# tinh2044/SCAttenNet

Measured on AMD Instinct MI355X. Metric: clips/sec fwd+bwd, (B=8,T=256,K=79,d=256) at 1/2/4/8 MI355X, higher is better.
Workload: dtype fp32; 1 GPU; cfg2: 4-stream SCA (mapping + 4x self / causal / cross-merge), B=8 T=256 K=79 d=256 H=16, fwd+bwd all params; clips_per_gpu=8, frames=256, joints=79, d_model=256, heads=16, layers=4, hipgraph=True, parallelism=dp1, devices=1

## Files before the change

### scattennet_amd/csrc/gemm.hip

```cpp
#include <stdlib.h>

#include <type_traits>
#include "common.h"
#include "../../include/scatten.h"

namespace {

constexpr int KPAD = 4;

struct GemmArgs {
  sca_gemm_problem p[SCA_GEMM_MAX_PROBLEMS];
  int splitk;
  float* ws;
  const unsigned long long* drop_off;
  long slab_off[SCA_GEMM_MAX_PROBLEMS];
  long bias_off[SCA_GEMM_MAX_PROBLEMS];
  unsigned* counters;
  int nprob;
  int flat;
  int tile_beg[SCA_GEMM_MAX_PROBLEMS + 1];
};

template <int BM_, int BN_, int WM_, int WN_, int BK_, int STAGES_>
struct Cfg {
// ... 1094 lines not shown
#pragma unroll
    for (int r = 0; r < 4; ++r)
#pragma unroll
      for (int i = 0; i < 4; ++i) {
        const int m = m0 + wm + 16 * g + 4 * r + i;
        if (m < P.M && ncol) {
          const f32x4 x = f32x4{acc[i][0][r], acc[i][1][r], acc[i][2][r], acc[i][3][r]} * alpha;
          const int off = (int)(((long)ks * MN + (long)m * P.N + n) * 4);
          if (fused_k) __builtin_amdgcn_raw_buffer_store_b128(*reinterpret_cast<const u32x4*>(&x), rs, off, 0, 16);
          else __builtin_amdgcn_raw_buffer_store_b128(*reinterpret_cast<const u32x4*>(&x), rs, off, 0, 0);
        }
      }
    if (!fused_k) return;
    asm volatile("s_waitcnt vmcnt(0)" ::: "memory");
    __syncthreads();
    unsigned* cnt = args.counters + (long)pid * gx * gy + (long)by * gx + bx;
    if (tid == 0)
      flag = __hip_atomic_fetch_add(cnt, 1u, __ATOMIC_RELAXED, __HIP_MEMORY_SCOPE_AGENT) == (unsigned)(splitk - 1);
    __syncthreads();
    if (!flag) return;
    if (tid == 0) __hip_atomic_store(cnt, 0u, __ATOMIC_RELAXED, __HIP_MEMORY_SCOPE_AGENT);
    __builtin_amdgcn_fence(__ATOMIC_ACQUIRE, "wavefront");
    if (P.bias_grad && bx == 0 && tid < TB_BM && m0 + tid < P.M) {
      float* bp = args.ws + args.bias_off[pid] + m0 + tid;
      float t = 0.f;
      for (int s2 = 0; s2 < splitk; ++s2)
        t += __hip_atomic_load(bp + (long)s2 * P.M, __ATOMIC_RELAXED, __HIP_MEMORY_SCOPE_AGENT);
      P.bias_grad[m0 + tid] = t * P.bias_grad_scale;
    }
    if (!ncol) return;
    DropMask dm;
    if (P.epi & SCA_EPI_DROPOUT) dm.init(P.drop_seed, P.drop_p, args.drop_off);
#pragma unroll 4
    for (int q = 0; q < 16; ++q) {
      const int m = m0 + wm + 16 * g + q;
      if (m >= P.M) continue;
      const long e = (long)m * P.N + n;
      f32x4 t = ld4_sc1(rs, e);
      for (int s2 = 1; s2 < splitk; ++s2) t += ld4_sc1(rs, s2 * MN + e);
      epilogue_piece(P, t, m, n, dm);
    }
    return;
  }
  if (!ncol) return;
  DropMask dm;
  if (P.epi & SCA_EPI_DROPOUT) dm.init(P.drop_seed, P.drop_p, args.drop_off);
#pragma unroll
  for (int r = 0; r < 4; ++r)
#pragma unroll
    for (int i = 0; i < 4; ++i) {
      const int m = m0 + wm + 16 * g + 4 * r + i;
      if (m < P.M)
        epilogue_piece(P, f32x4{acc[i][0][r], acc[i][1][r], acc[i][2][r], acc[i][3][r]} * alpha, m, n, dm);
    }
}

constexpr int NB_LD = TB_BK + 4;
constexpr int NB_OP = TB_BM * NB_LD;

template <bool INTER, int NPRE, bool B_KN, bool ILV = false, int TM = 128>
__global__ __launch_bounds__(256, 1) void gemm_ntb_kernel(const GemmArgs args) {
  constexpr int WT = TM / 2, NQ = WT / 16, NJ = TM / 16;
  constexpr int OP = TM * NB_LD;
  __shared__ __attribute__((aligned(16))) float lds[2 * OP];
  if constexpr (B_KN && SCA_CRIT_PRIO > 0) __builtin_amdgcn_s_setprio(SCA_CRIT_PRIO);

  const unsigned gx = gridDim.x, gy = gridDim.y;
  const unsigned nwg = gx * gy * gridDim.z;
  const unsigned orig = blockIdx.x + gx * (blockIdx.y + gy * blockIdx.z);
  const unsigned xcd = orig & 7, q8 = nwg >> 3, r8 = nwg & 7;
  const unsigned wgid = (xcd < r8 ? xcd * (q8 + 1) : r8 * (q8 + 1) + (xcd - r8) * q8) + (orig >> 3);
  const int bx = wgid % gx, by = (wgid / gx) % gy, pid = wgid / (gx * gy);
  const sca_gemm_problem& P = args.p[pid];
  const int m0 = by * TM, n0 = bx * TM;
  if (m0 >= P.M || n0 >= P.N) return;

  const int tid = threadIdx.x, lane = tid & 63, wave = tid >> 6;
  const int kg = lane >> 4, li = lane & 15;
  const int wm = (wave >> 1) * WT, wn = (wave & 1) * WT;
  const int nseg = P.nseg;
  const int it0 = P.seg[0].K / TB_BK, it1 = nseg > 1 ? P.seg[1].K / TB_BK : 0;
  const int nit = it0 + it1 + (nseg > 2 ? P.seg[2].K / TB_BK : 0);

  const int srow = tid >> 4, sk4 = 4 * (tid & 15);
  f32x4 st[2 * NJ];
  auto load = [&](int it) {
    int s = 0, lit = it;
    if (lit >= it0) {
      lit -= it0;
      s = 1;
      if (lit >= it1) {
        lit -= it1;
        s = 2;
      }
    }
    const sca_gemm_seg& G = P.seg[s];
    const __amdgpu_buffer_rsrc_t ra = __builtin_amdgcn_make_buffer_rsrc(
        const_cast<float*>(G.A), 0, (int)(((long)(P.M - 1) * G.lda + G.K) * 4), 0x00020000);
    const __amdgpu_buffer_rsrc_t rb = __builtin_amdgcn_make_buffer_rsrc(
        const_cast<float*>(G.B), 0,
        (int)((B_KN ? (long)(G.K - 1) * G.ldb + P.N : (long)(P.N - 1) * G.ldb + G.K) * 4), 0x00020000);
#pragma unroll
    for (int j = 0; j < NJ; ++j) {
      st[j] = tb_load(ra, (int)(((long)min(m0 + srow + 16 * j, P.M - 1) * G.lda + sk4) * 4), lit * TB_BK * 4);
      if constexpr (B_KN) {
        const int b = NJ * wave + j;
        const int k = 16 * (b & 3) + li, c4 = 4 * (4 * (b >> 2) + kg);
        st[NJ + j] = tb_load(rb, (int)(((long)k * G.ldb + min(n0 + c4, P.N - 4)) * 4), lit * TB_BK * G.ldb * 4);
      } else {
        st[NJ + j] = tb_load(rb, (int)(((long)min(n0 + srow + 16 * j, P.N - 1) * G.ldb + sk4) * 4), lit * TB_BK * 4);
      }
    }
  };
  float* wbase = lds + srow * NB_LD + sk4;
  auto store = [&]() {
#pragma unroll
    for (int j = 0; j < NJ; ++j) {
      st4(wbase + j * 16 * NB_LD, st[j]);
      if constexpr (B_KN) {
        const int b = NJ * wave + j;
        const int k = 16 * (b & 3) + li, c4 = 4 * (4 * (b >> 2) + kg);
#pragma unroll
        for (int q = 0; q < 4; ++q) lds[OP + (c4 + q) * NB_LD + k] = st[NJ + j][q];
      } else {
        st4(wbase + OP + j * 16 * NB_LD, st[NJ + j]);
      }
    }
  };

  f32x4 acc[NQ][NQ];
#pragma unroll
  for (int i = 0; i < NQ; ++i)
#pragma unroll
    for (int j = 0; j < NQ; ++j) acc[i][j] = f32x4{0.f, 0.f, 0.f, 0.f};

  const float* ra_lds = lds + (wm + li) * NB_LD + 4 * kg;
  const float* rb_lds = lds + OP + (wn + li) * NB_LD + 4 * kg;
  auto iter = [&](auto wr_c, auto ld_c, int it) {
    constexpr bool WR = decltype(wr_c)::value, LD = decltype(ld_c)::value;
    f32x4 a[4][NQ], b[4][NQ];
#pragma unroll
    for (int kc = 0; kc < 4; ++kc)
#pragma unroll
      for (int q = 0; q < NQ; ++q) {
        a[kc][q] = ld4(ra_lds + 16 * q * NB_LD + 16 * kc);
        b[kc][q] = ld4(rb_lds + 16 * q * NB_LD + 16 * kc);
      }
    auto steps = [&](int t0, int t1) {
#pragma unroll
      for (int t = t0; t < t1; ++t)
#pragma unroll
        for (int i = 0; i < NQ; ++i)
#pragma unroll
          for (int j = 0; j < NQ; ++j) acc[i][j] = mfma16(a[t >> 2][i][t & 3], b[t >> 2][j][t & 3], acc[i][j]);
    };
    steps(0, NPRE);
    if constexpr (ILV) ilv_read<0, 8, NQ, NPRE * NQ * NQ / 8>();
    if constexpr (INTER) __builtin_amdgcn_sched_barrier(0);
    __syncthreads();
    if constexpr (INTER) __builtin_amdgcn_sched_barrier(0);
    if constexpr (WR) {
      store();
      if constexpr (LD) load(it + 2);
    }
    steps(NPRE, 16);
    if constexpr (ILV && WR) ilv_store<0, 2 * NJ, B_KN ? 3 : 1, (16 - NPRE) * NQ * NQ / (2 * NJ)>();
    __syncthreads();
  };
  load(0);
  store();
  if (nit > 1) load(1);
  __syncthreads();
  int it = 0;
#pragma unroll 1
  for (; it + 2 < nit; ++it) iter(std::true_type{}, std::true_type{}, it);
  if (it + 1 < nit) iter(std::true_type{}, std::false_type{}, it++);
  if (it < nit) iter(std::false_type{}, std::false_type{}, it);

  constexpr int LR = WT / 4;
  float* img = lds + wave * WT * NB_LD;
  const float alpha = P.seg[0].alpha;
#pragma unroll
  for (int i = 0; i < NQ; ++i)
#pragma unroll
    for (int j = 0; j < NQ; ++j)
#pragma unroll
      for (int r = 0; r < 4; ++r) img[(16 * i + 4 * kg + r) * NB_LD + 16 * j + li] = acc[i][j][r] * alpha;
  __builtin_amdgcn_fence(__ATOMIC_RELEASE, "wavefront");
  __builtin_amdgcn_wave_barrier();
  __builtin_amdgcn_fence(__ATOMIC_ACQUIRE, "wavefront");
  const int n = n0 + wn + 4 * (lane % LR);
  if (n >= P.N) return;
  DropMask dm;
  if (P.epi & SCA_EPI_DROPOUT) dm.init(P.drop_seed, P.drop_p, args.drop_off);
#pragma unroll 4
  for (int q = 0; q < WT * LR / 64; ++q) {
    const int rho = lane / LR + (64 / LR) * q, m = m0 + wm + rho;
    if (m < P.M) epilogue_piece(P, ld4(img + rho * NB_LD + 4 * (lane % LR)), m, n, dm);
  }
}

constexpr int LR_SMEM = (32 + 256) * 68 * 4;
template <bool B_KN>
__device__ __forceinline__ void ln_rows_reg(const sca_gemm_problem& P, int m0, float* lds, f32x4 (&acc)[2][2]) {
  constexpr int LD = 68, NPRE = 4;
  const int tid = threadIdx.x, lane = tid & 63, wave = tid >> 6, kg = lane >> 4, li = lane & 15;
  float* Ai = lds;
  float* Bi = lds + 32 * LD;
  const int nseg = P.nseg;
  const int it0 = P.seg[0].K / 64, it1 = nseg > 1 ? P.seg[1].K / 64 : 0;
  const int nit = it0 + it1 + (nseg > 2 ? P.seg[2].K / 64 : 0);
  const int arow = tid >> 4, ak4 = 4 * (tid & 15);
  f32x4 st[9];
  auto load = [&](int it) {
    int sg = 0, lit = it;
    if (lit >= it0) {
      lit -= it0;
      sg = 1;
      if (lit >= it1) {
        lit -= it1;
        sg = 2;
      }
    }
    const sca_gemm_seg& G = P.seg[sg];
    const __amdgpu_buffer_rsrc_t ra = __builtin_amdgcn_make_buffer_rsrc(
        const_cast<float*>(G.A), 0, (int)(((long)(P.M - 1) * G.lda + G.K) * 4), 0x00020000);
    const __amdgpu_buffer_rsrc_t rb = __builtin_amdgcn_make_buffer_rsrc(
        const_cast<float*>(G.B), 0,
        (int)((B_KN ? (long)(G.K - 1) * G.ldb + P.N : (long)(P.N - 1) * G.ldb + G.K) * 4), 0x00020000);
    st[0] = tb_load(ra, (int)(((long)min(m0 + arow, P.M - 1) * G.lda + ak4) * 4), lit * 256);
#pragma unroll
    for (int j = 0; j < 8; ++j) {
      if constexpr (B_KN) {
        const int b = 8 * wave + j, k = 16 * (b & 3) + li, c4 = 4 * (4 * (b >> 2) + kg);
        st[1 + j] = tb_load(rb, (k * G.ldb + c4) * 4, lit * 64 * G.ldb * 4);
      } else {
        st[1 + j] = tb_load(rb, ((arow + 32 * j) * G.ldb + ak4) * 4, lit * 256);
      }
    }
  };
  auto store = [&]() {
    st4(Ai + arow * LD + ak4, st[0]);
#pragma unroll
    for (int j = 0; j < 8; ++j) {
      if constexpr (B_KN) {
        const int b = 8 * wave + j, k = 16 * (b & 3) + li, c4 = 4 * (4 * (b >> 2) + kg);
#pragma unroll
        for (int q = 0; q < 4; ++q) Bi[(c4 + q) * LD + k] = st[1 + j][q];
      } else {
        st4(Bi + (arow + 32 * j) * LD + ak4, st[1 + j]);
      }
    }
  };
#pragma unroll
  for (int i = 0; i < 2; ++i)
#pragma unroll
    for (int j = 0; j < 2; ++j) acc[i][j] = f32x4{0.f, 0.f, 0.f, 0.f};
  const float* ra_lds = Ai + li * LD + 4 * kg;
  const float* rb_lds = Bi + (32 * wave + li) * LD + 4 * kg;
  auto iter = [&](auto wr_c, auto ld_c, int it) {
    constexpr bool WR = decltype(wr_c)::value, LDN = decltype(ld_c)::value;
    f32x4 a[4][2], b[4][2];
#pragma unroll
    for (int kc = 0; kc < 4; ++kc)
#pragma unroll
      for (int q = 0; q < 2; ++q) {
        a[kc][q] = ld4(ra_lds + 16 * q * LD + 16 * kc);
        b[kc][q] = ld4(rb_lds + 16 * q * LD + 16 * kc);
      }
    auto steps = [&](int t0, int t1) {
#pragma unroll
      for (int t = t0; t < t1; ++t)
#pragma unroll
        for (int i = 0; i < 2; ++i)
#pragma unroll
          for (int j = 0; j < 2; ++j) acc[i][j] = mfma16(a[t >> 2][i][t & 3], b[t >> 2][j][t & 3], acc[i][j]);
    };
    steps(0, NPRE);
    ilv_read<0, 4, 4, NPRE>();
    __builtin_amdgcn_sched_barrier(0);
    __syncthreads();
    __builtin_amdgcn_sched_barrier(0);
    if constexpr (WR) {
      store();
      if constexpr (LDN) load(it + 2);
    }
    steps(NPRE, 16);
    if constexpr (WR) ilv_store<0, 9, B_KN ? 4 : 1, 5>();
    __syncthreads();
  };
  if (nit > 0) {
    load(0);
    store();
    if (nit > 1) load(1);
    __syncthreads();
  }
  int it = 0;
#pragma unroll 1
  for (; it + 2 < nit; ++it) iter(std::true_type{}, std::true_type{}, it);
  if (it + 1 < nit) iter(std::true_type{}, std::false_type{}, it++);
  if (it < nit) iter(std::false_type{}, std::false_type{}, it);
}

bool ln_reg_ok(const sca_gemm_problem& P, bool b_kn) {
  const long lim = (1L << 31) - 1;
  for (int s = 0; s < P.nseg; ++s) {
    const sca_gemm_seg& G = P.seg[s];
    if (G.K % 64 || G.K == 0) return false;
    if (((long)P.M * G.lda + G.K) * 4 > lim) return false;
    if ((b_kn ? (long)G.K * G.ldb + P.N : (long)P.N * G.ldb + G.K) * 4 > lim) return false;
  }
  return true;
}

bool ln_reg_default() {
  static const bool on = !(getenv("SCA_LNREG") && atoi(getenv("SCA_LNREG")) == 0);
  return on;
}
bool lnb_r3_default() {
  static const bool on = getenv("SCA_LNB_R3") && atoi(getenv("SCA_LNB_R3")) == 1;
  return on;
}

constexpr int LG_BN = 256, GL_A32 = 32, GL_A16 = 16;
constexpr int LG_B_BYTES = LG_BN * GL_BK * 4;
constexpr int LG_VS = LG_BN + 8;

template <int BM>
struct LgCfg {
  static constexpr int S = BM == 32 ? 3 : 2;
  static constexpr int A_BYTES = BM * GL_BK * 4;
  static constexpr int STAGE = A_BYTES + LG_B_BYTES;
  static constexpr int A_PIECES = BM / 8;
  static constexpr int NW = BM == 32 ? 8 : 4;
  static constexpr int BPW = 32 / NW;
};

constexpr int LG_A2_LD = 260;
constexpr int LG_A2_OFF = 2 * LG_B_BYTES;
constexpr int LG_SCR_OFF = LG_A2_OFF + 32 * LG_A2_LD * 4;
constexpr int LG_CH_SMEM = LG_SCR_OFF + 8 * 32 * EPI_LD * 4;
constexpr int LR_A2_OFF = 256 * 68 * 4;
constexpr int LR_SCR_OFF = LR_A2_OFF + 32 * LG_A2_LD * 4;
constexpr int LR_CH_SMEM = LR_SCR_OFF + 8 * 32 * EPI_LD * 4;

struct GemmLnArgs {
  sca_gemm_problem p[SCA_GEMM_LN_MAX_PROBLEMS];
  sca_gemm_ln_problem ln[SCA_GEMM_LN_MAX_PROBLEMS];
  float eps;
  const unsigned long long* drop_off;
  int rot;
};

__device__ __forceinline__ const float* lg_src(const float* base, int ld, int row0, int nrows, int pc, int lane) {
  const int r = 8 * pc + (lane >> 3);
  const int ks = (lane & 7) ^ gl_swz(r);
  return base + (long)min(row0 + r, nrows - 1) * ld + 4 * ks;
}

__device__ __forceinline__ f32x4 lg_slot(const char* img, int r, int slot) {
  return *(const f32x4*)(img + r * 128 + 16 * (slot ^ gl_swz(r)));
}

__device__ __forceinline__ f32x4 chain_bias(const sca_gemm_chain_pass& Q, int nb, int lane) {
  return Q.bias ? ld4(Q.bias + nb + 4 * (lane & 7)) : f32x4{0.f, 0.f, 0.f, 0.f};
}

__device__ __forceinline__ void chain_rows(const sca_gemm_chain_pass& Q, const f32x4 (&v)[4], int mb, int M, int nb,
                                           int lane, f32x4 bias) {
  const int n = nb + 4 * (lane & 7);
#pragma unroll
  for (int i = 0; i < 4; ++i) {
    const int m = mb + (lane >> 3) + 8 * i;
    if (m >= M) continue;
    f32x4 o = (v[i] + bias) * Q.post_scale;
    if (Q.epi & SCA_EPI_GELU) {
      st4g(Q.aux_out + (long)m * Q.ldo + n, o);
#pragma unroll
      for (int j = 0; j < 4; ++j) o[j] = gelu_erf(o[j]);
    }
    st4g(Q.C + (long)m * Q.ldc + n, o);
  }
}

template <int BM, bool CH, int NC, bool REG = false>
__global__ __launch_bounds__(LgCfg<BM>::NW * 64) void gemm_ln_kernel(const GemmLnArgs args) {
  using CF = LgCfg<BM>;
  constexpr int S = CF::S;
  constexpr int VS = NC * LG_BN + 8;
  constexpr int NROW = NC * LG_BN;
  static_assert(!CH || (BM == 32 && LG_CH_SMEM >= S * CF::STAGE && 32 * LG_VS * 4 <= LG_A2_OFF), "LDS map");
  static_assert(NC == 1 || (NC == 2 && BM == 32 && !CH && 32 * VS * 4 <= S * CF::STAGE), "LDS map (NC = 2)");
  static_assert(!REG || (BM == 32 && NC == 1 && LR_SMEM <= S * CF::STAGE), "LDS map (REG)");
  static_assert(!(REG && CH) || (32 * LG_VS * 4 <= LR_A2_OFF && LR_CH_SMEM <= 160 * 1024), "LDS map (REG, chained)");
  constexpr int A2OFF = REG ? LR_A2_OFF : LG_A2_OFF, SCROFF = REG ? LR_SCR_OFF : LG_SCR_OFF;
  __shared__ __attribute__((aligned(1024))) char smem[CH ? (REG ? LR_CH_SMEM : LG_CH_SMEM) : S * CF::STAGE];
  const unsigned gx = gridDim.x;
  const unsigned nwg = gx * gridDim.z;
  const unsigned orig = blockIdx.x + gx * blockIdx.z;
  const unsigned xcd = orig & 7, q8 = nwg >> 3, r8 = nwg & 7;
  const unsigned wgid = (xcd < r8 ? xcd * (q8 + 1) : r8 * (q8 + 1) + (xcd - r8) * q8) + (orig >> 3);
  const int pid = wgid / gx, bx = wgid % gx;
  const sca_gemm_problem& P = args.p[pid];
  const sca_gemm_ln_problem& LN = args.ln[pid];
  const int m0 = bx * BM;
  if (m0 >= P.M) return;
#ifdef SCA_GEMM_STAMPS
  const unsigned stamp_id = wgid;
#define SCA_LN_STAMP(slot) \
  if (threadIdx.x == 0 && stamp_id < STAMP_MAX) g_stamps[stamp_id][slot] = __builtin_amdgcn_s_memrealtime()
#else
#define SCA_LN_STAMP(slot) \
  do {                     \
  } while (0)
#endif
  SCA_LN_STAMP(0);
  const int lane = threadIdx.x & 63, wave = threadIdx.x >> 6;
  const sca_gemm_seg& G = P.seg[0];
  const int total = G.K / GL_BK;
  const int ttot = NC * total;

  const bool has_a = wave < CF::A_PIECES;
  const float* pa = lg_src(G.A, G.lda, m0, P.M, has_a ? wave : 0, lane);
  constexpr int BPW = CF::BPW;
  const float* pb[2] = {lg_src(G.B, G.ldb, 0, P.N, BPW * wave, lane),
                        lg_src(G.B, G.ldb, 0, P.N, BPW * wave + 1, lane)};
  const long pstep = 16L * G.ldb;
  auto dma = [&](int t, int stage) {
    char* base = smem + stage * CF::STAGE;
    const int half = NC == 2 && t >= total ? 1 : 0;
    const long kk = (long)(t - half * total) * GL_BK;
    const long hoff = (long)half * LG_BN * G.ldb;
    if (has_a) gl_dma(pa + kk, base + wave * GL_PIECE);
#pragma unroll
    for (int c = 0; c < BPW; ++c)
      gl_dma(pb[c & 1] + (c >> 1) * pstep + hoff + kk, base + CF::A_BYTES + (BPW * wave + c) * GL_PIECE);
  };

  constexpr int RPW = BM / CF::NW;
  const int n = 4 * lane;
  f32x4 rin[RPW][NC];
#pragma unroll
  for (int i = 0; i < RPW; ++i) {
    const int m = min(m0 + RPW * wave + i, P.M - 1);
#pragma unroll
    for (int c = 0; c < NC; ++c) rin[i][c] = ld4((P.resid ? P.resid + (long)m * P.ldr : LN.gamma) + LG_BN * c + n);
  }
  const f32x4 zero = {0.f, 0.f, 0.f, 0.f};
  f32x4 bias4[NC], gam[NC], bet[NC];
#pragma unroll
  for (int c = 0; c < NC; ++c) {
    bias4[c] = P.bias ? ld4(P.bias + LG_BN * c + n) : zero;
    gam[c] = ld4(LN.gamma + LG_BN * c + n);
    bet[c] = ld4(LN.beta + LG_BN * c + n);
  }
  float* V = reinterpret_cast<float*>(smem);
  const float alpha = G.alpha;
  if constexpr (REG) {
    f32x4 acc[2][2];
    ln_rows_reg<false>(P, m0, V, acc);
    SCA_LN_STAMP(1);
    const int li = lane & 15, kg = lane >> 4;
#pragma unroll
    for (int i = 0; i < 2; ++i)
#pragma unroll
      for (int j = 0; j < 2; ++j)
#pragma unroll
        for (int r = 0; r < 4; ++r) V[(16 * i + 4 * kg + r) * VS + 32 * wave + 16 * j + li] = acc[i][j][r] * alpha;
  } else if constexpr (BM == 32) {
    f32x16 acc[NC];
#pragma unroll
    for (int c = 0; c < NC; ++c)
#pragma unroll
      for (int r = 0; r < 16; ++r) acc[c][r] = 0.f;
#pragma unroll
    for (int i = 0; i < S - 1; ++i)
      if (i < ttot) dma(i, i);
    auto slice = [&](int t, f32x16& ac) {
      if (t + S - 2 < ttot) {
        if (has_a) gl_wait_vm<(BPW + 1) * (S - 2)>();
        else gl_wait_vm<BPW * (S - 2)>();
      } else {
        gl_wait_vm<0>();
      }
      __builtin_amdgcn_s_barrier();
      __builtin_amdgcn_sched_barrier(0);
      if (t + S - 1 < ttot) dma(t + S - 1, (t + S - 1) % S);
      const char* As = smem + (t % S) * CF::STAGE;
      const char* Bs = As + CF::A_BYTES;
      f32x4 fa[4], fb[4];
#pragma unroll
      for (int g = 0; g < 4; ++g) {
        fa[g] = gl_frag<true>(As, 0, g, lane);
        fb[g] = gl_frag<true>(Bs, 32 * wave, g, lane);
      }
#pragma unroll
      for (int g = 0; g < 4; ++g)
#pragma unroll
        for (int j = 0; j < 4; ++j) ac = mfma32(fa[g][j], fb[g][j], ac);
    };
    for (int t = 0; t < total; ++t) slice(t, acc[0]);
    if constexpr (NC == 2)
      for (int t = total; t < ttot; ++t) slice(t, acc[1]);
    __syncthreads();
    SCA_LN_STAMP(1);
    const int col = lane & 31, rowh = 4 * (lane >> 5);
#pragma unroll
    for (int c = 0; c < NC; ++c)
#pragma unroll
      for (int r = 0; r < 16; ++r)
        V[((r & 3) + 8 * (r >> 2) + rowh) * VS + LG_BN * c + 32 * wave + col] = acc[c][r] * alpha;
  } else {
    f32x4 acc[4];
#pragma unroll
    for (int j = 0; j < 4; ++j) acc[j] = f32x4{0.f, 0.f, 0.f, 0.f};
    const int li = lane & 15, grp = lane >> 4;
    if (total > 0) dma(0, 0);
    for (int t = 0; t < total; ++t) {
      gl_wait_vm<0>();
      __builtin_amdgcn_s_barrier();
      __builtin_amdgcn_sched_barrier(0);
      if (t + 1 < total) dma(t + 1, (t + 1) % S);
      const char* As = smem + (t % S) * CF::STAGE;
      const char* Bs = As + CF::A_BYTES;
#pragma unroll
      for (int c = 0; c < 2; ++c) {
        const f32x4 af = lg_slot(As, li, 4 * c + grp);
        f32x4 bf[4];
#pragma unroll
        for (int j = 0; j < 4; ++j) bf[j] = lg_slot(Bs, 64 * wave + 16 * j + li, 4 * c + grp);
#pragma unroll
        for (int r = 0; r < 4; ++r)
#pragma unroll
          for (int j = 0; j < 4; ++j) acc[j] = mfma16(af[r], bf[j][r], acc[j]);
      }
    }
    __syncthreads();
#pragma unroll
    for (int j = 0; j < 4; ++j)
#pragma unroll
      for (int r = 0; r < 4; ++r) V[(4 * grp + r) * VS + 64 * wave + 16 * j + li] = acc[j][r] * alpha;
  }
  __syncthreads();
  __builtin_amdgcn_s_waitcnt(0x0F70);

  DropMask dm;
  const bool drop = (P.epi & SCA_EPI_DROPOUT) != 0;
  if (drop) dm.init(P.drop_seed, P.drop_p, args.drop_off);
  const float invN = 1.0f / NROW;
  f32x4 v[RPW][NC];
  float s[RPW];
#pragma unroll
  for (int i = 0; i < RPW; ++i) {
    const int lr = RPW * wave + i, m = min(m0 + lr, P.M - 1);
    s[i] = 0.f;
#pragma unroll
    for (int c = 0; c < NC; ++c) {
      f32x4 x = (ld4(&V[lr * VS + LG_BN * c + n]) + bias4[c]) * P.post_scale;
      if (drop) {
#pragma unroll
        for (int j = 0; j < 4; ++j)
          x[j] = dm.apply((uint32_t)m * (uint32_t)P.N + (uint32_t)(LG_BN * c + n + j), x[j]);
      }
      if (P.resid) x += rin[i][c];
      v[i][c] = x;
      s[i] += (x[0] + x[1]) + (x[2] + x[3]);
    }
  }
  const int nit2 = CH && REG ? 4 * LN.npass : 0;
  f32x4 st2[8];
  auto load2 = [&](int u) {
    int q = (u >> 2) + (args.rot && LN.npass > 0 ? bx % LN.npass : 0);
    q = q >= LN.npass ? q - LN.npass : q;
    const sca_gemm_chain_pass& Q = LN.pass[q];
    const __amdgpu_buffer_rsrc_t rb = __builtin_amdgcn_make_buffer_rsrc(
        const_cast<float*>(Q.B), 0, (int)(((long)(LG_BN - 1) * Q.ldb + LG_BN) * 4), 0x00020000);
    const int t = threadIdx.x;
#pragma unroll
    for (int j = 0; j < 8; ++j)
      st2[j] = tb_load(rb, ((32 * (t >> 6) + ((t & 63) >> 4) + 4 * j) * Q.ldb + 4 * (t & 15)) * 4, (u & 3) * 256);
  };
  auto store2 = [&]() {
    float* Bi = reinterpret_cast<float*>(smem);
    const int t = threadIdx.x;
#pragma unroll
    for (int j = 0; j < 8; ++j) st4(Bi + (32 * (t >> 6) + ((t & 63) >> 4) + 4 * j) * 68 + 4 * (t & 15), st2[j]);
  };
  if constexpr (CH && REG) {
    if (nit2 > 0) load2(0);
  }
  const int nsl = CH && !REG ? 8 * LN.npass : 0;
  const int prot = CH && args.rot && LN.npass > 0 ? bx % LN.npass : 0;
  auto pass_of = [&](int u) {
    int q = (u >> 3) + prot;
    return q >= LN.npass ? q - LN.npass : q;
  };
  auto dma2 = [&](int u, int stage) {
    const sca_gemm_chain_pass& Q = LN.pass[pass_of(u)];
    char* base = smem + stage * LG_B_BYTES;
    const long k0 = 32L * (u & 7);
#pragma unroll
    for (int c = 0; c < 4; ++c)
      gl_dma(lg_src(Q.B, Q.ldb, 0, LG_BN, 4 * wave + c, lane) + k0, base + (4 * wave + c) * GL_PIECE);
  };
  if constexpr (CH) {
    __syncthreads();
    if constexpr (REG) {
      if (nit2 > 0) store2();
      if (nit2 > 1) load2(1);
    } else {
      if (nsl > 0) dma2(0, 0);
      if (nsl > 1) dma2(1, 1);
    }
  }
#pragma unroll
  for (int o = 32; o > 0; o >>= 1)
#pragma unroll
    for (int i = 0; i < RPW; ++i) s[i] += __shfl_xor(s[i], o, 64);
  float q[RPW];
#pragma unroll
  for (int i = 0; i < RPW; ++i) {
    q[i] = 0.f;
#pragma unroll
    for (int c = 0; c < NC; ++c) {
      const f32x4 dv = v[i][c] - s[i] * invN;
      q[i] += (dv[0] * dv[0] + dv[1] * dv[1]) + (dv[2] * dv[2] + dv[3] * dv[3]);
    }
  }
#pragma unroll
  for (int o = 32; o > 0; o >>= 1)
#pragma unroll
    for (int i = 0; i < RPW; ++i) q[i] += __shfl_xor(q[i], o, 64);
#pragma unroll
  for (int i = 0; i < RPW; ++i) {
    const int lr = RPW * wave + i, m = m0 + lr;
    const float mean = s[i] * invN;
    const float rstd = 1.0f / sqrtf(q[i] * invN + args.eps);
#pragma unroll
    for (int c = 0; c < NC; ++c) {
      const f32x4 y = (v[i][c] - mean) * rstd * gam[c] + bet[c];
      if (CH) st4(reinterpret_cast<float*>(smem + A2OFF) + lr * LG_A2_LD + n, y);
      if (m < P.M) {
        st4g(P.C + (long)m * P.ldc + LG_BN * c + n, v[i][c]);
        st4g(LN.y + (long)m * NROW + LG_BN * c + n, y);
      }
    }
    if (m < P.M) {
      if (lane == 0) {
        st1g(LN.mean + m, mean);
        st1g(LN.rstd + m, rstd);
      }
    }
  }
  if constexpr (CH && REG) {
    const float* A2 = reinterpret_cast<const float*>(smem + A2OFF);
    const float* Bi = reinterpret_cast<const float*>(smem);
    float* scratch = reinterpret_cast<float*>(smem + SCROFF) + wave * 32 * EPI_LD;
    const int li = lane & 15, kg = lane >> 4;
    const int prot2 = args.rot && LN.npass > 0 ? bx % LN.npass : 0;
    f32x4 acc2[2][2];
#pragma unroll
    for (int i = 0; i < 2; ++i)
#pragma unroll
      for (int j = 0; j < 2; ++j) acc2[i][j] = f32x4{0.f, 0.f, 0.f, 0.f};
    lds_barrier();
    SCA_LN_STAMP(2);
    f32x4 cbias = f32x4{0.f, 0.f, 0.f, 0.f};
    auto iter2 = [&](auto wr_c, auto ld_c, int u) {
      constexpr bool WR = decltype(wr_c)::value, LDN = decltype(ld_c)::value;
      if ((u & 3) == 0) {
        int pq0 = (u >> 2) + prot2;
        pq0 = pq0 >= LN.npass ? pq0 - LN.npass : pq0;
        cbias = chain_bias(LN.pass[pq0], 32 * wave, lane);
      }
      f32x4 a[4][2], b[4][2];
#pragma unroll
      for (int kc = 0; kc < 4; ++kc)
#pragma unroll
        for (int q = 0; q < 2; ++q) {
          a[kc][q] = ld4(A2 + (16 * q + li) * LG_A2_LD + 64 * (u & 3) + 16 * kc + 4 * kg);
          b[kc][q] = ld4(Bi + (32 * wave + 16 * q + li) * 68 + 16 * kc + 4 * kg);
        }
      auto steps = [&](int t0, int t1) {
#pragma unroll
        for (int t = t0; t < t1; ++t)
#pragma unroll
          for (int i = 0; i < 2; ++i)
#pragma unroll
            for (int j = 0; j < 2; ++j) acc2[i][j] = mfma16(a[t >> 2][i][t & 3], b[t >> 2][j][t & 3], acc2[i][j]);
      };
      steps(0, 4);
      ilv_read<0, 4, 4, 4>();
      __builtin_amdgcn_sched_barrier(0);
      __builtin_amdgcn_fence(__ATOMIC_RELEASE, "wavefront");
      __builtin_amdgcn_wave_barrier();
      __builtin_amdgcn_fence(__ATOMIC_ACQUIRE, "wavefront");
      __builtin_amdgcn_sched_barrier(0);
      if constexpr (WR) {
        store2();
        if constexpr (LDN) load2(u + 2);
      }
      steps(4, 16);
      if constexpr (WR) ilv_store<0, 8, 1, 6>();
      if ((u & 3) == 3) {
#pragma unroll
        for (int i = 0; i < 2; ++i)
#pragma unroll
          for (int j = 0; j < 2; ++j)
#pragma unroll
            for (int r = 0; r < 4; ++r) scratch[(16 * i + 4 * kg + r) * EPI_LD + 16 * j + li] = acc2[i][j][r];
        __builtin_amdgcn_fence(__ATOMIC_RELEASE, "wavefront");
        __builtin_amdgcn_wave_barrier();
        __builtin_amdgcn_fence(__ATOMIC_ACQUIRE, "wavefront");
        f32x4 rows[4];
#pragma unroll
        for (int q = 0; q < 4; ++q) rows[q] = ld4(scratch + ((lane >> 3) + 8 * q) * EPI_LD + 4 * (lane & 7));
        int pq = (u >> 2) + prot2;
        pq = pq >= LN.npass ? pq - LN.npass : pq;
        chain_rows(LN.pass[pq], rows, m0, P.M, 32 * wave, lane, cbias);
        if (u == 3) SCA_LN_STAMP(3);
#pragma unroll
        for (int i = 0; i < 2; ++i)
#pragma unroll
          for (int j = 0; j < 2; ++j) acc2[i][j] = f32x4{0.f, 0.f, 0.f, 0.f};
        __builtin_amdgcn_fence(__ATOMIC_RELEASE, "wavefront");
        __builtin_amdgcn_wave_barrier();
        __builtin_amdgcn_fence(__ATOMIC_ACQUIRE, "wavefront");
      }
      __builtin_amdgcn_fence(__ATOMIC_RELEASE, "wavefront");
      __builtin_amdgcn_wave_barrier();
      __builtin_amdgcn_fence(__ATOMIC_ACQUIRE, "wavefront");
    };
    int u = 0;
#pragma unroll 1
    for (; u + 2 < nit2; ++u) iter2(std::true_type{}, std::true_type{}, u);
    if (u + 1 < nit2) iter2(std::true_type{}, std::false_type{}, u++);
    if (u < nit2) iter2(std::false_type{}, std::false_type{}, u);
  }
  if constexpr (CH && !REG) {
    const float* A2 = reinterpret_cast<const float*>(smem + LG_A2_OFF);
    float* scratch = reinterpret_cast<float*>(smem + LG_SCR_OFF) + wave * 32 * EPI_LD;
    const int col = lane & 31, h = lane >> 5;
    f32x16 acc2;
#pragma unroll
    for (int r = 0; r < 16; ++r) acc2[r] = 0.f;
    lds_barrier();
    SCA_LN_STAMP(2);
    const bool full = m0 + BM <= P.M;
    for (int u = 0; u < nsl; ++u) {
      if (!full) {
        gl_wait_vm<0>();
      } else if (u == 0) {
        if (nsl > 1) gl_wait_vm<20>();
        else gl_wait_vm<16>();
      } else if ((u & 7) == 0) {
        if (LN.pass[pass_of(u - 1)].epi & SCA_EPI_GELU) gl_wait_vm<8>();
        else gl_wait_vm<4>();
      } else {
        gl_wait_vm<0>();
      }
      __builtin_amdgcn_s_barrier();
      __builtin_amdgcn_sched_barrier(0);
      if (u >= 1 && u + 1 < nsl) dma2(u + 1, (u + 1) & 1);
      const int t = u & 7;
      const char* Bs = smem + (u & 1) * LG_B_BYTES;
      f32x4 fa[4], fb[4];
#pragma unroll
      for (int g = 0; g < 4; ++g) {
        fa[g] = ld4(A2 + col * LG_A2_LD + 32 * t + 8 * g + 4 * h);
        fb[g] = gl_frag<true>(Bs, 32 * wave, g, lane);
      }
#pragma unroll
      for (int g = 0; g < 4; ++g)
#pragma unroll
        for (int j = 0; j < 4; ++j) acc2 = mfma32(fa[g][j], fb[g][j], acc2);
      if (t == 7) {
        f32x4 rows[4];
        acc_to_rows(acc2, scratch, lane, rows);
        chain_rows(LN.pass[pass_of(u)], rows, m0, P.M, 32 * wave, lane, chain_bias(LN.pass[pass_of(u)], 32 * wave, lane));
#pragma unroll
        for (int r = 0; r < 16; ++r) acc2[r] = 0.f;
        if (u == 7) SCA_LN_STAMP(3);
      }
    }
  }
#ifdef SCA_GEMM_STAMPS
  asm volatile("s_waitcnt vmcnt(0)" ::: "memory");
  __syncthreads();
#endif
  SCA_LN_STAMP(4);
#undef SCA_LN_STAMP
}

constexpr int LB_BM = 32, LB_S = 3;
constexpr int LB_BROW = 1056;
constexpr int LB_A_BYTES = LB_BM * GL_BK * 4;
constexpr int LB_STAGE = LB_A_BYTES + GL_BK * LB_BROW;
constexpr int LB_B2 = GL_BK * LB_BROW;
constexpr int LB_A2_LD = 260;
constexpr int LB_A2_OFF = 2 * LB_B2;
constexpr int LB_RED_OFF = LB_A2_OFF + LB_BM * LB_A2_LD * 4;
constexpr int LB_SMEM = LB_RED_OFF + 2 * 8 * 256 * 4 > LB_S * LB_STAGE ? LB_RED_OFF + 2 * 8 * 256 * 4
                                                                         : LB_S * LB_STAGE;
constexpr int LB_B3_OFF = LB_SMEM;
constexpr int LB_SMEM3 = LB_B3_OFF + LB_B2;

struct GemmLnbArgs {
  sca_gemm_problem p[SCA_GEMM_MAX_PROBLEMS];
  sca_gemm_lnb_problem ln[SCA_GEMM_MAX_PROBLEMS];
};

template <int NC, bool REG = false, bool R3 = false>
__global__ __launch_bounds__(512) void gemm_lnb_kernel(const GemmLnbArgs args) {
  if constexpr (SCA_CRIT_PRIO > 0) __builtin_amdgcn_s_setprio(SCA_CRIT_PRIO);
  static_assert(!R3 || (NC == 1 && LB_SMEM3 <= 160 * 1024), "LDS map (R3)");
  __shared__ __attribute__((aligned(1024))) char smem[R3 ? LB_SMEM3 : LB_SMEM];
  constexpr int VS = NC * LG_BN + 8, NROW = NC * LG_BN;
  constexpr int RED_OFF = NC == 1 ? LB_RED_OFF : LB_BM * VS * 4;
  static_assert(LB_B2 >= LB_BM * LG_VS * 4 && LB_RED_OFF + 2 * 8 * LG_BN * 4 <= LB_SMEM, "LDS map");
  static_assert(NC == 1 || RED_OFF + 2 * 8 * NROW * 4 <= LB_SMEM, "LDS map (NC = 2)");
  static_assert(!REG || (NC == 1 && LR_SMEM <= LB_SMEM), "LDS map (REG)");
  const unsigned gx = gridDim.x;
  const unsigned nwg = gx * gridDim.z;
  const unsigned orig = blockIdx.x + gx * blockIdx.z;
  const unsigned xcd = orig & 7, q8 = nwg >> 3, r8 = nwg & 7;
  const unsigned wgid = (xcd < r8 ? xcd * (q8 + 1) : r8 * (q8 + 1) + (xcd - r8) * q8) + (orig >> 3);
  const int pid = wgid / gx, bx = wgid % gx;
  const sca_gemm_problem& P = args.p[pid];
  const sca_gemm_lnb_problem& LN = args.ln[pid];
  const int m0 = bx * LB_BM;
  if (m0 >= P.M) return;
  const int lane = threadIdx.x & 63, wave = threadIdx.x >> 6;
  const bool has_a = wave < 4;

  int seg_n[SCA_GEMM_MAX_SEGS];
  int total = 0;
#pragma unroll
  for (int s = 0; s < SCA_GEMM_MAX_SEGS; ++s) {
    seg_n[s] = s < P.nseg ? P.seg[s].K / GL_BK : 0;
    total += seg_n[s];
  }
  const int ttot = NC * total;
  int iseg = -1, tseg0 = 0, tend = 0;
  const float* pa = nullptr;
  const float* pb = nullptr;
  long ldb = 0;
  auto dma = [&](int t, int stage) {
    const int half = NC == 2 && t >= total ? 1 : 0;
    if (NC == 2 && t == total) {
      iseg = -1;
      tend = 0;
    }
    t -= half * total;
    while (t >= tend) {
      ++iseg;
      tseg0 = tend;
      tend += seg_n[iseg];
      const sca_gemm_seg& G = P.seg[iseg];
      pa = lg_src(G.A, G.lda, m0, P.M, has_a ? wave : 0, lane);
      ldb = G.ldb;
      pb = G.B + (long)(4 * wave) * ldb + 4 * lane + LG_BN * half;
    }
    const long k0 = (long)(t - tseg0) * GL_BK;
    char* base = smem + stage * LB_STAGE;
    if (has_a) gl_dma(pa + k0, base + wave * GL_PIECE);
#pragma unroll
    for (int c = 0; c < 4; ++c) gl_dma(pb + (k0 + c) * ldb, base + LB_A_BYTES + (4 * wave + c) * LB_BROW);
  };

  constexpr int RPW = LB_BM / 8;
  const int n = 4 * lane;
  f32x4 xin[RPW][NC], rin[RPW][NC], gam[NC];
  float mu[RPW], rs[RPW];
#pragma unroll
  for (int c = 0; c < NC; ++c) gam[c] = ld4(LN.gamma + LG_BN * c + n);
#pragma unroll
  for (int i = 0; i < RPW; ++i) {
    const int m = min(m0 + RPW * wave + i, P.M - 1);
#pragma unroll
    for (int c = 0; c < NC; ++c) {
      const int nc = LG_BN * c + n;
      xin[i][c] = ld4(LN.x + (long)m * NROW + nc);
      if (LN.tab) xin[i][c] += ld4(LN.tab + (long)(m % LN.tab_T + 2) * NROW + nc);
      rin[i][c] = ld4((P.resid ? P.resid + (long)m * P.ldr : LN.gamma) + nc);
    }
    mu[i] = LN.mean[m];
    rs[i] = LN.rstd[m];
  }
  f32x16 acc[NC];
#pragma unroll
  for (int c = 0; c < NC; ++c)
#pragma unroll
    for (int r = 0; r < 16; ++r) acc[c][r] = 0.f;
  const int col = lane & 31, h = lane >> 5;
  f32x4 racc[2][2];
  if constexpr (REG) {
    ln_rows_reg<true>(P, m0, reinterpret_cast<float*>(smem), racc);
  } else {
#pragma unroll
  for (int i = 0; i < LB_S - 1; ++i)
    if (i < ttot) dma(i, i);
  auto slice = [&](int t, f32x16& ac) {
    if (t + LB_S - 2 < ttot) {
      if (has_a) gl_wait_vm<5 * (LB_S - 2)>();
      else gl_wait_vm<4 * (LB_S - 2)>();
    } else {
      gl_wait_vm<0>();
    }
    __builtin_amdgcn_s_barrier();
    __builtin_amdgcn_sched_barrier(0);
    if (t + LB_S - 1 < ttot) dma(t + LB_S - 1, (t + LB_S - 1) % LB_S);
    const char* As = smem + (t % LB_S) * LB_STAGE;
    const float* Bf = reinterpret_cast<const float*>(As + LB_A_BYTES);
    f32x4 fa[4], fb[4];
#pragma unroll
    for (int g = 0; g < 4; ++g) {
      fa[g] = gl_frag<true>(As, 0, g, lane);
#pragma unroll
      for (int j = 0; j < 4; ++j) fb[g][j] = Bf[(8 * g + 4 * h + j) * (LB_BROW / 4) + 32 * wave + col];
    }
#pragma unroll
    for (int g = 0; g < 4; ++g)
#pragma unroll
      for (int j = 0; j < 4; ++j) ac = mfma32(fa[g][j], fb[g][j], ac);
  };
  for (int t = 0; t < total; ++t) slice(t, acc[0]);
  if constexpr (NC == 2)
    for (int t = total; t < ttot; ++t) slice(t, acc[1]);
  }
  __syncthreads();
  float* V = reinterpret_cast<float*>(smem);
  const float alpha = P.seg[0].alpha;
  const int rowh = 4 * h;
  if constexpr (REG) {
    const int li = lane & 15, kg = lane >> 4;
#pragma unroll
    for (int i = 0; i < 2; ++i)
#pragma unroll
      for (int j = 0; j < 2; ++j)
#pragma unroll
        for (int r = 0; r < 4; ++r) V[(16 * i + 4 * kg + r) * VS + 32 * wave + 16 * j + li] = racc[i][j][r] * alpha;
  } else {
#pragma unroll
  for (int c = 0; c < NC; ++c)
#pragma unroll
    for (int r = 0; r < 16; ++r)
      V[((r & 3) + 8 * (r >> 2) + rowh) * VS + LG_BN * c + 32 * wave + col] = acc[c][r] * alpha;
  }
  __syncthreads();

  __builtin_amdgcn_s_waitcnt(0x0F70);
  const float invN = 1.0f / NROW;
  f32x4 g[RPW][NC], xh[RPW][NC];
  float s1[RPW], s2[RPW];
#pragma unroll
  for (int i = 0; i < RPW; ++i) {
    s1[i] = s2[i] = 0.f;
#pragma unroll
    for (int c = 0; c < NC; ++c) {
      g[i][c] = ld4(&V[(RPW * wave + i) * VS + LG_BN * c + n]);
      if (P.resid) g[i][c] += rin[i][c];
      xh[i][c] = (xin[i][c] - mu[i]) * rs[i];
      const f32x4 gg = g[i][c] * gam[c];
      s1[i] += (gg[0] + gg[1]) + (gg[2] + gg[3]);
      const f32x4 ggx = gg * xh[i][c];
      s2[i] += (ggx[0] + ggx[1]) + (ggx[2] + ggx[3]);
    }
  }
  const bool chain = NC == 1 && LN.wo != nullptr;
  const int npass = chain ? max(LN.npass, 1) : 0;
  const long ldw = LN.ldw ? LN.ldw : (long)LG_BN * npass;
  const float* pw = LN.wo + (long)(4 * wave) * ldw + 4 * lane;
  auto stage_at = [&](int stage) { return smem + (R3 && stage == 2 ? LB_B3_OFF : stage * LB_B2); };
  auto dma2 = [&](int u, int stage) {
    const float* src = pw + (u >> 3) * LG_BN + (long)(32 * (u & 7)) * ldw;
#pragma unroll
    for (int c = 0; c < 4; ++c) gl_dma(src + c * ldw, stage_at(stage) + (4 * wave + c) * LB_BROW);
  };
  if (chain) {
    __syncthreads();
    dma2(0, 0);
    dma2(1, 1);
  }
#pragma unroll
  for (int o = 32; o > 0; o >>= 1)
#pragma unroll
    for (int i = 0; i < RPW; ++i) {
      s1[i] += __shfl_xor(s1[i], o, 64);
      s2[i] += __shfl_xor(s2[i], o, 64);
    }
  f32x4 pg[NC], pbsum[NC];
#pragma unroll
  for (int c = 0; c < NC; ++c) pg[c] = pbsum[c] = f32x4{0.f, 0.f, 0.f, 0.f};
  float* A2 = reinterpret_cast<float*>(smem + LB_A2_OFF);
#pragma unroll
  for (int i = 0; i < RPW; ++i) {
    const int lr = RPW * wave + i, m = m0 + lr;
#pragma unroll
    for (int c = 0; c < NC; ++c) {
      const f32x4 d = (g[i][c] * gam[c] - s1[i] * invN - xh[i][c] * (s2[i] * invN)) * rs[i];
      if (chain) st4(A2 + lr * LB_A2_LD + n, d);
      if (m < P.M) {
        st4g(P.C + (long)m * P.ldc + LG_BN * c + n, g[i][c]);
        st4g(LN.dx + (long)m * NROW + LG_BN * c + n, d);
        pg[c] += g[i][c] * xh[i][c];
        pbsum[c] += g[i][c];
      }
    }
  }
  float* red = reinterpret_cast<float*>(smem + RED_OFF);
#pragma unroll
  for (int c = 0; c < NC; ++c) {
    st4(red + wave * NROW + LG_BN * c + n, pg[c]);
    st4(red + (8 + wave) * NROW + LG_BN * c + n, pbsum[c]);
  }
  lds_barrier();
  const long nblk = (P.M + LB_BM - 1) / LB_BM;
#pragma unroll
  for (int c = 0; c < NC; ++c) {
    const int e = threadIdx.x + 512 * c;
    const int cc = e % NROW, which = e / NROW;
    const float* rr = red + which * 8 * NROW + cc;
    const float sum = (((rr[0] + rr[NROW]) + (rr[2 * NROW] + rr[3 * NROW])) +
                       ((rr[4 * NROW] + rr[5 * NROW]) + (rr[6 * NROW] + rr[7 * NROW])));
    st1g(LN.partial + (which * nblk + bx) * NROW + cc, sum);
  }
  if (!chain) return;

  const bool dgelu = LN.aux != nullptr;
  f32x16 acc2;
#pragma unroll
  for (int r = 0; r < 16; ++r) acc2[r] = 0.f;
  const int nsl = 8 * npass;
  const bool full = m0 + LB_BM <= P.M;
  const long n2 = (long)(npass - 1) * LG_BN + 32 * wave + 4 * (lane & 7);
  float axe[16];
  f32x4 axr[4];
  for (int u = 0; u < nsl; ++u) {
    const bool last_pass = (u >> 3) == npass - 1;
    if constexpr (R3) {
// ... 710 lines not shown
```

Baseline: 1849 clips/s.

## Load chained-pass B fragments directly into registers, skipping LDS staging

In the register-path chained LN GEMM, the second GEMM's B tiles now go from global memory (buffer loads) straight into double-buffered MFMA-fragment registers instead of being staged through LDS with store/ld4 round trips. The loop is restructured into groups of four k-steps per pass with a new sched_group_barrier interleave, and the B staging area is dropped from the LDS map. The LDS allocation is padded to a fixed size (default on), which likely limits blocks per CU. This removes LDS write/read traffic and barriers per step, at the cost of more live registers and uncoalesced or strided global loads per lane.

```diff
diff --git a/scattennet_amd/csrc/gemm.hip b/scattennet_amd/csrc/gemm.hip
--- a/scattennet_amd/csrc/gemm.hip
+++ b/scattennet_amd/csrc/gemm.hip
@@ -1420,6 +1420,20 @@
   if (it < nit) iter(std::false_type{}, std::false_type{}, it);
 }
 
+template <int G>
+__device__ __forceinline__ void ilv_chain_direct() {
+  if constexpr (G < 4) {
+    if constexpr (G == 0) __builtin_amdgcn_sched_group_barrier(0x100, 4, 0);
+    __builtin_amdgcn_sched_group_barrier(0x020, 1, 0);
+    __builtin_amdgcn_sched_group_barrier(0x008, 6, 0);
+    if constexpr (G < 2) __builtin_amdgcn_sched_group_barrier(0x100, 2, 0);
+    __builtin_amdgcn_sched_group_barrier(0x008, 5, 0);
+    __builtin_amdgcn_sched_group_barrier(0x020, 1, 0);
+    __builtin_amdgcn_sched_group_barrier(0x008, 5, 0);
+    ilv_chain_direct<G + 1>();
+  }
+}
+
 bool ln_reg_ok(const sca_gemm_problem& P, bool b_kn) {
   const long lim = (1L << 31) - 1;
   for (int s = 0; s < P.nseg; ++s) {
@@ -1458,9 +1472,14 @@
 constexpr int LG_A2_OFF = 2 * LG_B_BYTES;
 constexpr int LG_SCR_OFF = LG_A2_OFF + 32 * LG_A2_LD * 4;
 constexpr int LG_CH_SMEM = LG_SCR_OFF + 8 * 32 * EPI_LD * 4;
-constexpr int LR_A2_OFF = 256 * 68 * 4;
+#ifndef SCA_LR_CH_PAD
+#define SCA_LR_CH_PAD 1
+#endif
+constexpr int LR_A2_OFF = 32 * LG_VS * 4;
 constexpr int LR_SCR_OFF = LR_A2_OFF + 32 * LG_A2_LD * 4;
-constexpr int LR_CH_SMEM = LR_SCR_OFF + 8 * 32 * EPI_LD * 4;
+constexpr int LR_CH_NATURAL = LR_SCR_OFF + 8 * 32 * EPI_LD * 4;
+constexpr int LR_CH_SMEM = SCA_LR_CH_PAD ? 143872 : LR_CH_NATURAL;
+static_assert(LR_CH_SMEM >= LR_CH_NATURAL && LR_CH_SMEM >= LR_SMEM, "LDS map (REG, chained)");
 
 struct GemmLnArgs {
   sca_gemm_problem p[SCA_GEMM_LN_MAX_PROBLEMS];
@@ -1686,8 +1705,10 @@
     }
   }
   const int nit2 = CH && REG ? 4 * LN.npass : 0;
-  f32x4 st2[8];
-  auto load2 = [&](int u) {
+  f32x4 bd2[2][4][2];
+  auto load2 = [&](auto s_c, int u) {
+    constexpr int s = decltype(s_c)::value;
+    u = __builtin_amdgcn_readfirstlane(min(u, nit2 - 1));
     int q = (u >> 2) + (args.rot && LN.npass > 0 ? bx % LN.npass : 0);
     q = q >= LN.npass ? q - LN.npass : q;
     const sca_gemm_chain_pass& Q = LN.pass[q];
@@ -1695,17 +1716,14 @@
         const_cast<float*>(Q.B), 0, (int)(((long)(LG_BN - 1) * Q.ldb + LG_BN) * 4), 0x00020000);
     const int t = threadIdx.x;
 #pragma unroll
-    for (int j = 0; j < 8; ++j)
-      st2[j] = tb_load(rb, ((32 * (t >> 6) + ((t & 63) >> 4) + 4 * j) * Q.ldb + 4 * (t & 15)) * 4, (u & 3) * 256);
-  };
-  auto store2 = [&]() {
-    float* Bi = reinterpret_cast<float*>(smem);
-    const int t = threadIdx.x;
-#pragma unroll
-    for (int j = 0; j < 8; ++j) st4(Bi + (32 * (t >> 6) + ((t & 63) >> 4) + 4 * j) * 68 + 4 * (t & 15), st2[j]);
+    for (int kc = 0; kc < 4; ++kc)
+#pragma unroll
+      for (int qq = 0; qq < 2; ++qq)
+        bd2[s][kc][qq] = tb_load(rb, ((32 * (t >> 6) + 16 * qq + (t & 15)) * Q.ldb + 16 * kc + 4 * ((t & 63) >> 4)) * 4,
+                                 (u & 3) * 256);
   };
   if constexpr (CH && REG) {
-    if (nit2 > 0) load2(0);
+    if (nit2 > 0) load2(std::integral_constant<int, 0>{}, 0);
   }
   const int nsl = CH && !REG ? 8 * LN.npass : 0;
   const int prot = CH && args.rot && LN.npass > 0 ? bx % LN.npass : 0;
@@ -1721,15 +1739,10 @@
     for (int c = 0; c < 4; ++c)
       gl_dma(lg_src(Q.B, Q.ldb, 0, LG_BN, 4 * wave + c, lane) + k0, base + (4 * wave + c) * GL_PIECE);
   };
-  if constexpr (CH) {
+  if constexpr (CH && !REG) {
     __syncthreads();
-    if constexpr (REG) {
-      if (nit2 > 0) store2();
-      if (nit2 > 1) load2(1);
-    } else {
-      if (nsl > 0) dma2(0, 0);
-      if (nsl > 1) dma2(1, 1);
-    }
+    if (nsl > 0) dma2(0, 0);
+    if (nsl > 1) dma2(1, 1);
   }
 #pragma unroll
   for (int o = 32; o > 0; o >>= 1)
@@ -1772,7 +1785,6 @@
   }
   if constexpr (CH && REG) {
     const float* A2 = reinterpret_cast<const float*>(smem + A2OFF);
-    const float* Bi = reinterpret_cast<const float*>(smem);
     float* scratch = reinterpret_cast<float*>(smem + SCROFF) + wave * 32 * EPI_LD;
     const int li = lane & 15, kg = lane >> 4;
     const int prot2 = args.rot && LN.npass > 0 ? bx % LN.npass : 0;
@@ -1783,77 +1795,54 @@
       for (int j = 0; j < 2; ++j) acc2[i][j] = f32x4{0.f, 0.f, 0.f, 0.f};
     lds_barrier();
     SCA_LN_STAMP(2);
-    f32x4 cbias = f32x4{0.f, 0.f, 0.f, 0.f};
-    auto iter2 = [&](auto wr_c, auto ld_c, int u) {
-      constexpr bool WR = decltype(wr_c)::value, LDN = decltype(ld_c)::value;
-      if ((u & 3) == 0) {
-        int pq0 = (u >> 2) + prot2;
-        pq0 = pq0 >= LN.npass ? pq0 - LN.npass : pq0;
-        cbias = chain_bias(LN.pass[pq0], 32 * wave, lane);
-      }
-      f32x4 a[4][2], b[4][2];
+    auto iter2 = [&](auto s_c, int u) {
+      constexpr int s = decltype(s_c)::value;
+      f32x4 a[4][2];
 #pragma unroll
       for (int kc = 0; kc < 4; ++kc)
 #pragma unroll
-        for (int q = 0; q < 2; ++q) {
-          a[kc][q] = ld4(A2 + (16 * q + li) * LG_A2_LD + 64 * (u & 3) + 16 * kc + 4 * kg);
-          b[kc][q] = ld4(Bi + (32 * wave + 16 * q + li) * 68 + 16 * kc + 4 * kg);
-        }
-      auto steps = [&](int t0, int t1) {
-#pragma unroll
-        for (int t = t0; t < t1; ++t)
-#pragma unroll
-          for (int i = 0; i < 2; ++i)
-#pragma unroll
-            for (int j = 0; j < 2; ++j) acc2[i][j] = mfma16(a[t >> 2][i][t & 3], b[t >> 2][j][t & 3], acc2[i][j]);
-      };
-      steps(0, 4);
-      ilv_read<0, 4, 4, 4>();
+        for (int q = 0; q < 2; ++q) a[kc][q] = ld4(A2 + (16 * q + li) * LG_A2_LD + 64 * (u & 3) + 16 * kc + 4 * kg);
+      load2(std::integral_constant<int, s ^ 1>{}, u + 1);
+#pragma unroll
+      for (int t = 0; t < 16; ++t)
+#pragma unroll
+        for (int i = 0; i < 2; ++i)
+#pragma unroll
+          for (int j = 0; j < 2; ++j) acc2[i][j] = mfma16(a[t >> 2][i][t & 3], bd2[s][t >> 2][j][t & 3], acc2[i][j]);
+      ilv_chain_direct<0>();
       __builtin_amdgcn_sched_barrier(0);
+    };
+#pragma unroll 1
+    for (int u = 0; u < nit2; u += 4) {
+      int pq = (u >> 2) + prot2;
+      pq = pq >= LN.npass ? pq - LN.npass : pq;
+      const f32x4 cbias = chain_bias(LN.pass[pq], 32 * wave, lane);
+      iter2(std::integral_constant<int, 0>{}, u);
+      iter2(std::integral_constant<int, 1>{}, u + 1);
+      iter2(std::integral_constant<int, 0>{}, u + 2);
+      iter2(std::integral_constant<int, 1>{}, u + 3);
+#pragma unroll
+      for (int i = 0; i < 2; ++i)
+#pragma unroll
+        for (int j = 0; j < 2; ++j)
+#pragma unroll
+          for (int r = 0; r < 4; ++r) scratch[(16 * i + 4 * kg + r) * EPI_LD + 16 * j + li] = acc2[i][j][r];
       __builtin_amdgcn_fence(__ATOMIC_RELEASE, "wavefront");
       __builtin_amdgcn_wave_barrier();
       __builtin_amdgcn_fence(__ATOMIC_ACQUIRE, "wavefront");
-      __builtin_amdgcn_sched_barrier(0);
-      if constexpr (WR) {
-        store2();
-        if constexpr (LDN) load2(u + 2);
-      }
-      steps(4, 16);
-      if constexpr (WR) ilv_store<0, 8, 1, 6>();
-      if ((u & 3) == 3) {
-#pragma unroll
-        for (int i = 0; i < 2; ++i)
-#pragma unroll
-          for (int j = 0; j < 2; ++j)
-#pragma unroll
-            for (int r = 0; r < 4; ++r) scratch[(16 * i + 4 * kg + r) * EPI_LD + 16 * j + li] = acc2[i][j][r];
-        __builtin_amdgcn_fence(__ATOMIC_RELEASE, "wavefront");
-        __builtin_amdgcn_wave_barrier();
-        __builtin_amdgcn_fence(__ATOMIC_ACQUIRE, "wavefront");
-        f32x4 rows[4];
-#pragma unroll
-        for (int q = 0; q < 4; ++q) rows[q] = ld4(scratch + ((lane >> 3) + 8 * q) * EPI_LD + 4 * (lane & 7));
-        int pq = (u >> 2) + prot2;
-        pq = pq >= LN.npass ? pq - LN.npass : pq;
-        chain_rows(LN.pass[pq], rows, m0, P.M, 32 * wave, lane, cbias);
-        if (u == 3) SCA_LN_STAMP(3);
-#pragma unroll
-        for (int i = 0; i < 2; ++i)
-#pragma unroll
-          for (int j = 0; j < 2; ++j) acc2[i][j] = f32x4{0.f, 0.f, 0.f, 0.f};
-        __builtin_amdgcn_fence(__ATOMIC_RELEASE, "wavefront");
-        __builtin_amdgcn_wave_barrier();
-        __builtin_amdgcn_fence(__ATOMIC_ACQUIRE, "wavefront");
-      }
+      f32x4 rows[4];
+#pragma unroll
+      for (int q = 0; q < 4; ++q) rows[q] = ld4(scratch + ((lane >> 3) + 8 * q) * EPI_LD + 4 * (lane & 7));
+      chain_rows(LN.pass[pq], rows, m0, P.M, 32 * wave, lane, cbias);
+      if (u == 0) SCA_LN_STAMP(3);
+#pragma unroll
+      for (int i = 0; i < 2; ++i)
+#pragma unroll
+        for (int j = 0; j < 2; ++j) acc2[i][j] = f32x4{0.f, 0.f, 0.f, 0.f};
       __builtin_amdgcn_fence(__ATOMIC_RELEASE, "wavefront");
       __builtin_amdgcn_wave_barrier();
       __builtin_amdgcn_fence(__ATOMIC_ACQUIRE, "wavefront");
-    };
-    int u = 0;
-#pragma unroll 1
-    for (; u + 2 < nit2; ++u) iter2(std::true_type{}, std::true_type{}, u);
-    if (u + 1 < nit2) iter2(std::true_type{}, std::false_type{}, u++);
-    if (u < nit2) iter2(std::false_type{}, std::false_type{}, u);
+    }
   }
   if constexpr (CH && !REG) {
     const float* A2 = reinterpret_cast<const float*>(smem + LG_A2_OFF);
```

After: 1858 clips/s (median of 6 runs). Within noise of the previous version (+0.5%).
